# tarepan/QuickVC-official

Measured on AMD Instinct MI355X. Metric: audio samples/sec (16 kHz, 5 s utterances, batch 32 per GPU, whole hot path), higher is better.
Workload: dtype bf16x; 1 GPU; batch=32 offline VC, 5 s 16 kHz utterances, 1xMI355X per rank (BASELINE.json configs[2]); batch_per_gpu=32, frames=250, samples_per_utterance=80000, hipgraph=True, parallel_resblock_branches=False, parallelism=utterance-sharded x1, no per-step collective, batches_in_flight=2

## Files before the change

quickvc-official_amd/build.py:

```python
from __future__ import annotations

import os
import subprocess
import sys
from concurrent.futures import ThreadPoolExecutor

PKG = os.path.dirname(os.path.abspath(__file__))
ROOT = os.path.dirname(PKG)
CSRC = os.path.join(PKG, "csrc")
OBJ = os.path.join(PKG, "csrc", "_obj")
LIB = os.path.join(PKG, "libqvc_hip.so")
IO_LIB = os.path.join(PKG, "libqvc_io.so")
EMU_DIR = os.path.join(ROOT, "oracle", "_build")
EMU_LIB = os.path.join(EMU_DIR, "libqvc_emu.so")
HIPCC = os.environ.get("HIPCC", "/opt/rocm/bin/hipcc")
ARCH = "gfx950"

SOURCES = ["qvc_conv_f16.hip", "qvc_conv_bf16.hip", "qvc_wn2.hip", "qvc_chain.hip", "qvc_small.hip", "qvc_spk.hip", "qvc_mel.hip", "qvc_api.hip", "qvc_pack.cpp"]
HEADERS = ["qvc_plan.h", "qvc_kernels.h", "qvc_conv_impl.h", "qvc_wn2_impl.h", "qvc_chain_impl.h", "qvc_post_tail_impl.h", "qvc_tail_impl.h", "qvc_path.h", "qvc_stream.h", "qvc_pack_util.h", "qvc_launch_util.h"]


def _newer(target: str, deps) -> bool:
    if not os.path.exists(target):
        return False
    t = os.path.getmtime(target)
    return all(os.path.getmtime(d) <= t for d in deps)


def _run(cmd):
    res = subprocess.run(cmd, stdout=subprocess.PIPE, stderr=subprocess.STDOUT, text=True)
    if res.returncode != 0:
        raise RuntimeError("command failed: %s\n%s" % (" ".join(cmd), res.stdout))
    if "-c" in cmd and "-o" in cmd and cmd[cmd.index("-o") + 1].endswith(".o"):
        with open(cmd[cmd.index("-o") + 1][:-2] + ".remarks.txt", "w") as f:
            f.write(res.stdout)
    return res.stdout


def build_hip(force: bool = False, verbose: bool = False, variant: str = "") -> str:
    extra = {"": [], "sat": ["-DQVC_SATCOUNT"]}[variant]
    obj_dir = OBJ if not variant else os.path.join(OBJ, variant)
    lib = LIB if not variant else os.path.join(PKG, f"libqvc_hip_{variant}.so")
    os.makedirs(obj_dir, exist_ok=True)
    hdrs = [os.path.join(CSRC, h) for h in HEADERS] + [os.path.join(ROOT, "include", "qvc.h")]
    objs, jobs = [], []
    for src in SOURCES:
        s = os.path.join(CSRC, src)
        o = os.path.join(obj_dir, os.path.splitext(src)[0] + ".o")
        objs.append(o)
        if force or not _newer(o, [s] + hdrs):
            jobs.append([HIPCC, f"--offload-arch={ARCH}", "-O3", "-std=c++17", "-fPIC", "-Rpass-analysis=kernel-resource-usage"] + extra +
                        ["-c", s, "-o", o])
    if jobs:
        with ThreadPoolExecutor(max_workers=min(len(jobs), 6)) as ex:
            for out in ex.map(_run, jobs):
                if verbose and out.strip():
                    print(out)
    if jobs or not os.path.exists(lib):
        _run([HIPCC, f"--offload-arch={ARCH}", "-shared", "-fPIC", "-o", lib] + objs)
    return lib


def build_io(force: bool = False) -> str:
    src = os.path.join(CSRC, "qvc_io.cpp")
    hdr = os.path.join(ROOT, "include", "qvc_io.h")
    if force or not _newer(IO_LIB, [src, hdr]):
        _run(["g++", "-O2", "-std=c++17", "-fPIC", "-shared", "-pthread", "-o", IO_LIB, src])
    return IO_LIB


def build_emu(force: bool = False) -> str:
    os.makedirs(EMU_DIR, exist_ok=True)
    srcs = [os.path.join(ROOT, "oracle", "qvc_emu.cpp"), os.path.join(CSRC, "qvc_pack.cpp")]
    hdrs = [os.path.join(CSRC, h) for h in HEADERS] + [os.path.join(ROOT, "include", "qvc.h")]
    if force or not _newer(EMU_LIB, srcs + hdrs):
        _run(["g++", "-O2", "-std=c++17", "-fPIC", "-shared", "-o", EMU_LIB] + srcs)
    return EMU_LIB


if __name__ == "__main__":
    force = "--force" in sys.argv
    print(build_hip(force, verbose=True))
    print(build_hip(force, variant="sat"))
    print(build_io(force))
    print(build_emu(force))
```

quickvc-official_amd/csrc/qvc_conv_impl.h:

```cpp
#pragma once
#include <hip/hip_runtime.h>
#include <algorithm>
#include <type_traits>
#include <cstdlib>
#include "qvc_kernels.h"
#include "qvc_launch_util.h"

#ifndef QVC_SWZ_ROT
#define QVC_SWZ_ROT 1
#endif
namespace qvc {

typedef float f32x4 __attribute__((ext_vector_type(4)));
typedef _Float16 f16x8 __attribute__((ext_vector_type(8)));
typedef __bf16 bf16x8 __attribute__((ext_vector_type(8)));
typedef _Float16 f16x4 __attribute__((ext_vector_type(4)));
typedef __bf16 bf16x4 __attribute__((ext_vector_type(4)));

#ifdef QVC_SATCOUNT
static __device__ unsigned long long g_sat_count = 0;
#define QVC_SAT_READER(name)                                                                        \
  unsigned long long name(bool reset) {                                                             \
    unsigned long long v = 0, z = 0;                                                                \
    if (hipMemcpyFromSymbol(&v, HIP_SYMBOL(g_sat_count), 8) != hipSuccess) return ~0ull;            \
    if (reset && hipMemcpyToSymbol(HIP_SYMBOL(g_sat_count), &z, 8) != hipSuccess) return ~0ull;     \
    return v;                                                                                       \
  }
#endif

template <typename T> struct Op;
template <> struct Op<_Float16> {
  using frag = f16x8; using quad = f16x4;
  static __device__ __forceinline__ f32x4 mfma(frag a, frag b, f32x4 c) {
    return __builtin_amdgcn_mfma_f32_16x16x32_f16(a, b, c, 0, 0, 0);
  }
  static __device__ __forceinline__ _Float16 cvt(float f) {
#ifdef QVC_SATCOUNT
    if (__builtin_fabsf(f) > 65504.f) atomicAdd(&g_sat_count, 1ull);
#endif
    return (_Float16)__builtin_amdgcn_fmed3f(f, -65504.f, 65504.f);
  }
};
template <> struct Op<__bf16> {
  using frag = bf16x8; using quad = bf16x4;
  static __device__ __forceinline__ f32x4 mfma(frag a, frag b, f32x4 c) {
    return __builtin_amdgcn_mfma_f32_16x16x32_bf16(a, b, c, 0, 0, 0);
  }
  static __device__ __forceinline__ __bf16 cvt(float f) { return (__bf16)f; }
};

__device__ __forceinline__ float lrelu(float x, float slope) { return x > 0.f ? x : x * slope; }
__device__ __forceinline__ float fast_sigmoid(float x) {
  return __builtin_amdgcn_rcpf(1.f + __builtin_amdgcn_exp2f(-1.4426950408889634f * x));
}
__device__ __forceinline__ float fast_tanh(float x) {
  return 1.f - 2.f * __builtin_amdgcn_rcpf(__builtin_amdgcn_exp2f(2.8853900817779268f * x) + 1.f);
}

struct Swz { int sh, mask, rot; };
__device__ __forceinline__ Swz swz_mode(int cpr) {
  return (cpr & 15) == 0 ? Swz{0, QVC_SWZ_ROT ? 7 : 15, QVC_SWZ_ROT} : ((cpr & 7) == 0 ? Swz{0, 7, 0} : Swz{1, 3, 0});
}
__device__ __forceinline__ int swz(int row, Swz m) { return (row >> m.sh) & m.mask; }
__device__ __forceinline__ int rotc(int chunk, Swz m) {
  return m.rot ? ((chunk & ~15) | ((chunk & 1) << 3) | ((chunk >> 1) & 7)) : chunk;
}
template <typename B>
__device__ __forceinline__ B tile_at(B base, int row, int chunk, int rowbytes, Swz m) {
  return base + row * rowbytes + ((rotc(chunk, m) ^ swz(row, m)) << 4);
}

#define QVC_ZERO_ACC(acc) \
  _Pragma("unroll") for (auto& row_ : acc) { _Pragma("unroll") for (auto& e_ : row_) e_ = f32x4{0.f, 0.f, 0.f, 0.f}; }

__device__ __forceinline__ bool in_row(int ti, int Tlo, int Tin, int reflect, int& src) {
  if (reflect) { src = ti == Tlo ? Tlo + 1 : ti - 1; return ti >= Tlo && ti <= Tin; }
  src = ti;
  return ti >= Tlo && ti < Tin;
}

template <typename T>
__device__ __forceinline__ typename Op<T>::frag lrelu8(typename Op<T>::frag v, float slope) {
  typename Op<T>::frag r;
#pragma unroll
  for (int i = 0; i < 8; ++i) {
    const float f = (float)v[i];
    r[i] = (T)(f > 0.f ? f : f * slope);
  }
  return r;
}

template <>
__device__ __forceinline__ f16x8 lrelu8<_Float16>(f16x8 v, float slope) {
  f16x8 s;
#pragma unroll
  for (int i = 0; i < 8; ++i) s[i] = (_Float16)((float)v[i] * slope);
  return __builtin_elementwise_max(v, s);
}

template <typename T, typename TS>
__device__ __forceinline__ typename Op<T>::frag act8(typename Op<TS>::frag h, float slope) {
  if constexpr (std::is_same<T, TS>::value) {
    return lrelu8<T>(h, slope);
  } else {
    typename Op<T>::frag o;
#pragma unroll
    for (int e = 0; e < 8; ++e) o[e] = Op<T>::cvt(lrelu((float)h[e], slope));
    return o;
  }
}

template <typename T>
__device__ __forceinline__ typename Op<T>::frag cvt8(float4 v0, float4 v1) {
  using O = Op<T>;
  typename O::frag h;
  h[0] = O::cvt(v0.x); h[1] = O::cvt(v0.y); h[2] = O::cvt(v0.z); h[3] = O::cvt(v0.w);
  h[4] = O::cvt(v1.x); h[5] = O::cvt(v1.y); h[6] = O::cvt(v1.z); h[7] = O::cvt(v1.w);
  return h;
}
template <typename T>
__device__ __forceinline__ typename Op<T>::frag cvt8_lrelu(float4 v0, float4 v1, float slope) {
  return cvt8<T>(make_float4(lrelu(v0.x, slope), lrelu(v0.y, slope), lrelu(v0.z, slope), lrelu(v0.w, slope)),
                 make_float4(lrelu(v1.x, slope), lrelu(v1.y, slope), lrelu(v1.z, slope), lrelu(v1.w, slope)));
}

template <typename T>
__device__ __forceinline__ typename Op<T>::quad pack4_lrelu(f32x4 a, float4 b, float slope) {
  using O = Op<T>;
  typename O::quad h;
  h[0] = O::cvt(lrelu(a[0] + b.x, slope)); h[1] = O::cvt(lrelu(a[1] + b.y, slope));
  h[2] = O::cvt(lrelu(a[2] + b.z, slope)); h[3] = O::cvt(lrelu(a[3] + b.w, slope));
  return h;
}
template <typename T>
__device__ __forceinline__ typename Op<T>::quad pack4_res(f32x4 a, float4 b, typename Op<T>::quad r) {
  using O = Op<T>;
  typename O::quad h;
  h[0] = O::cvt(a[0] + b.x + (float)r[0]); h[1] = O::cvt(a[1] + b.y + (float)r[1]);
  h[2] = O::cvt(a[2] + b.z + (float)r[2]); h[3] = O::cvt(a[3] + b.w + (float)r[3]);
  return h;
}
template <typename T>
__device__ __forceinline__ typename Op<T>::frag pack8_lrelu(f32x4 a0, float4 b0, f32x4 a1, float4 b1, float slope) {
  const typename Op<T>::quad lo = pack4_lrelu<T>(a0, b0, slope), hi = pack4_lrelu<T>(a1, b1, slope);
  return __builtin_shufflevector(lo, hi, 0, 1, 2, 3, 4, 5, 6, 7);
}
template <typename T>
__device__ __forceinline__ typename Op<T>::frag pack8_res(f32x4 a0, float4 b0, f32x4 a1, float4 b1, typename Op<T>::frag r) {
  using quad = typename Op<T>::quad;
  const quad lo = pack4_res<T>(a0, b0, __builtin_shufflevector(r, r, 0, 1, 2, 3));
  const quad hi = pack4_res<T>(a1, b1, __builtin_shufflevector(r, r, 4, 5, 6, 7));
  return __builtin_shufflevector(lo, hi, 0, 1, 2, 3, 4, 5, 6, 7);
}

template <typename T>
__device__ __forceinline__ typename Op<T>::quad gate4(f32x4 t, f32x4 s, float4 bt, float4 bs) {
  using O = Op<T>;
  typename O::quad o;
  o[0] = O::cvt(fast_tanh(t[0] + bt.x) * fast_sigmoid(s[0] + bs.x));
  o[1] = O::cvt(fast_tanh(t[1] + bt.y) * fast_sigmoid(s[1] + bs.y));
  o[2] = O::cvt(fast_tanh(t[2] + bt.z) * fast_sigmoid(s[2] + bs.z));
  o[3] = O::cvt(fast_tanh(t[3] + bt.w) * fast_sigmoid(s[3] + bs.w));
  return o;
}

#ifndef QVC_PF_CONV
#define QVC_PF_CONV 3
#endif
#ifdef QVC_ABLATE
#define QVC_ABL(bit) ((QVC_ABLATE >> (bit)) & 1)
#else
#define QVC_ABL(bit) 0
#endif
#ifdef QVC_STAMP
#define QVC_ST(slot) do { if (st_ && lane == 0) st_[slot] = __builtin_amdgcn_s_memtime(); } while (0)
#else
#define QVC_ST(slot) ((void)0)
#endif
#ifndef QVC_PF_WN
#define QVC_PF_WN 3
#endif
#ifndef QVC_PF_STACK
#define QVC_PF_STACK 3
#endif

template <typename T, int MF, int kPF, int AS = MF>
__device__ __forceinline__ void gemm_prime(typename Op<T>::frag (&ar)[kPF + 1][MF], const typename Op<T>::frag* ap, int nIt) {
#pragma unroll
  for (int u = 0; u < kPF; ++u)
    if (u < nIt) {
#pragma unroll
      for (int m = 0; m < MF; ++m) ar[u][m] = ap[((size_t)u * AS + m) * 64];
    }
}

template <typename T, int MF, int NF, int kPF, int AS = MF>
__device__ __forceinline__ void gemm_loop_primed(f32x4 (&acc)[MF][NF], typename Op<T>::frag (&ar)[kPF + 1][MF],
                                                 const typename Op<T>::frag* ap, int nIt, int KS, int dil,
                                                 const char* tile, int rowbytes, Swz sm, int colrow, int lq) {
  using O = Op<T>;
  using frag = typename O::frag;
  constexpr int RING = kPF + 1;
  static_assert(RING % 2 == 0, "the B double buffer needs an even ring");
  frag bf[2][NF];
  const int nstride = 16 * rowbytes;
  int pf = kPF < nIt ? kPF : nIt;
  int tap = 0, ks = 0;
  auto read_b = [&](frag (&dst)[NF]) {
    const int row0 = tap * dil + colrow;
    const char* bp = tile + row0 * rowbytes + ((rotc(ks * 4 + lq, sm) ^ swz(row0, sm)) << 4);
#pragma unroll
    for (int n = 0; n < NF; ++n) dst[n] = *reinterpret_cast<const frag*>(bp + n * nstride);
    if (++ks == KS) { ks = 0; ++tap; }
  };
  if (nIt > 0) read_b(bf[0]);
  for (int it0 = 0; it0 < nIt; it0 += RING) {
#pragma unroll
    for (int u = 0; u < RING; ++u) {
      const int it = it0 + u;
      if (it < nIt) {
        if (it + kPF < nIt && !QVC_ABL(5)) {
#pragma unroll
          for (int m = 0; m < MF; ++m) ar[(u + kPF) % RING][m] = ap[((size_t)pf * AS + m) * 64];
          ++pf;
        }
        if (it + 1 < nIt && !QVC_ABL(6)) read_b(bf[(u + 1) & 1]);
        __builtin_amdgcn_sched_barrier(0);
#pragma unroll
        for (int n = 0; n < NF; ++n)
#pragma unroll
          for (int m = 0; m < MF; ++m) acc[m][n] = O::mfma(ar[u][m], bf[u & 1][n], acc[m][n]);
        __builtin_amdgcn_sched_barrier(0);
      }
    }
  }
}

template <typename T, int MF, int NF, int kPF, int AS = MF>
__device__ __forceinline__ void gemm_loop(f32x4 (&acc)[MF][NF], const typename Op<T>::frag* ap, int nIt, int KS, int dil,
                                          const char* tile, int rowbytes, Swz sm, int colrow, int lq) {
  typename Op<T>::frag ar[kPF + 1][MF];
  gemm_prime<T, MF, kPF, AS>(ar, ap, nIt);
  gemm_loop_primed<T, MF, NF, kPF, AS>(acc, ar, ap, nIt, KS, dil, tile, rowbytes, sm, colrow, lq);
}

template <typename T, typename TS, int NTHR, typename Put, typename Mid>
__device__ __forceinline__ void stage_stream_tile(const TS* xb, int C, int cpr, int total, int t_base, int Tlo, int Tb, float slope,
                                                  int tid, Put&& put, Mid&& loads_issued) {
  constexpr int kU = 16;
  const int rstep = NTHR / cpr, cstep = NTHR - rstep * cpr;
  for (int base = tid; base < total; base += NTHR * kU) {
    uint4 v[kU];
    const int r_0 = base / cpr, c_0 = base - r_0 * cpr;
    int r = r_0, c8 = c_0;
#pragma unroll
    for (int u = 0; u < kU; ++u) {
      const int idx = base + u * NTHR;
      const int ti = t_base + r;
      v[u] = make_uint4(0u, 0u, 0u, 0u);
      if (idx < total && ti >= Tlo && ti < Tb && c8 * 8 < C) v[u] = *reinterpret_cast<const uint4*>(xb + (size_t)ti * C + c8 * 8);
      c8 += cstep; r += rstep;
      if (c8 >= cpr) { c8 -= cpr; ++r; }
    }
    r = r_0; c8 = c_0;
    loads_issued(base == tid);
#pragma unroll
    for (int u = 0; u < kU; ++u) {
      const int idx = base + u * NTHR;
      if (idx < total) {
        typename Op<TS>::frag h; __builtin_memcpy(&h, &v[u], 16);
        put(r, c8, v[u], act8<T, TS>(h, slope));
      }
      c8 += cstep; r += rstep;
      if (c8 >= cpr) { c8 -= cpr; ++r; }
    }
  }
}

template <typename T, int MF, int NF, int WM, int EPI, bool CL = false>
__global__ __launch_bounds__(256) void conv_mfma_kernel(const ConvArgs a) {
  using O = Op<T>;
  using frag = typename O::frag;
  extern __shared__ __attribute__((aligned(16))) char smem[];
  constexpr int WN = kWaves / WM;
  constexpr int NT = WN * NF * 16;

  const int tid = threadIdx.x, lane = tid & 63;
  const int wave = __builtin_amdgcn_readfirstlane(tid >> 6);
  const int wm = wave % WM, wn = wave / WM;
  const int b = blockIdx.y;
  const int q0 = blockIdx.x * NT;
  const int R = NT + (a.taps - 1) * a.dil;
  const int rowbytes = a.CinP * 2;
  const int cpr = a.CinP >> 3;
  const Swz sm = swz_mode(cpr);
  const int t_base = q0 - a.left;
  const int Tin = ragged_len(a.rg, b, a.T_in);
  const int Tlo = ragged_lo(a.rg, b);
  if (a.rg.lens && t_base >= Tin + a.reflect) return;

  constexpr int kU = 4;
  if (a.x_kind == XK_F32_FM) {
    const float* xb = static_cast<const float*>(a.x) + (size_t)b * a.x_bs + a.x_c0;
    const float slope = a.slope_in;
    const int total = R * cpr;
    for (int base = tid; base < total; base += 256 * kU) {
      float4 v0[kU], v1[kU];
      int dst[kU];
#pragma unroll
      for (int u = 0; u < kU; ++u) {
        const int idx = base + u * 256;
        const int r = idx / cpr, c8 = idx - r * cpr;
        const int ti = t_base + r;
        int src;
        const bool ok = in_row(ti, Tlo, Tin, a.reflect, src) && idx < total && (c8 * 8 < a.Cin);
        v0[u] = make_float4(0.f, 0.f, 0.f, 0.f); v1[u] = v0[u];
        if (ok) {
          const float4* p = reinterpret_cast<const float4*>(xb + (size_t)src * a.x_ts + c8 * 8);
          v0[u] = p[0]; v1[u] = p[1];
        }
        dst[u] = idx < total ? tile_at(0, r, c8, rowbytes, sm) : -1;
      }
#pragma unroll
      for (int u = 0; u < kU; ++u) {
        if (dst[u] < 0) continue;
        *reinterpret_cast<frag*>(smem + dst[u]) = cvt8_lrelu<T>(v0[u], v1[u], slope);
      }
    }
  } else if (a.x_kind == XK_OP_FM && a.x2) {
    const size_t boff = (size_t)b * a.x_bs + a.x_c0;
    const T* xb = static_cast<const T*>(a.x) + boff;
    const T* xb2 = static_cast<const T*>(a.x2) + boff;
    const T* xb3 = static_cast<const T*>(a.x3) + boff;
    const float slope = a.slope_in;
    const int total = R * cpr;
    for (int base = tid; base < total; base += 256 * kU) {
      uint4 v1[kU], v2[kU], v3[kU];
      int dst[kU];
#pragma unroll
      for (int u = 0; u < kU; ++u) {
        const int idx = base + u * 256;
        const int r = idx / cpr, c8 = idx - r * cpr;
        const int ti = t_base + r;
        int src;
        const bool ok = in_row(ti, Tlo, Tin, a.reflect, src) && idx < total && (c8 * 8 < a.Cin);
        v1[u] = make_uint4(0u, 0u, 0u, 0u); v2[u] = v1[u]; v3[u] = v1[u];
        if (ok) {
          const size_t o = (size_t)src * a.x_ts + c8 * 8;
          v1[u] = *reinterpret_cast<const uint4*>(xb + o);
          v2[u] = *reinterpret_cast<const uint4*>(xb2 + o);
          v3[u] = *reinterpret_cast<const uint4*>(xb3 + o);
        }
        dst[u] = idx < total ? tile_at(0, r, c8, rowbytes, sm) : -1;
      }
#pragma unroll
      for (int u = 0; u < kU; ++u) {
        if (dst[u] < 0) continue;
        frag h1, h2, h3, h;
        __builtin_memcpy(&h1, &v1[u], 16); __builtin_memcpy(&h2, &v2[u], 16); __builtin_memcpy(&h3, &v3[u], 16);
#pragma unroll
        for (int i = 0; i < 8; ++i)
          h[i] = O::cvt(lrelu(((float)h1[i] + (float)h2[i] + (float)h3[i]) * (1.f / 3.f), slope));
        *reinterpret_cast<frag*>(smem + dst[u]) = h;
      }
    }
  } else if (a.x_kind == XK_OP_FM) {
    const T* xb = static_cast<const T*>(a.x) + (size_t)b * a.x_bs + a.x_c0;
    const int total = R * cpr;
    for (int base = tid; base < total; base += 256 * kU * 2) {
      uint4 v[kU * 2];
      int dst[kU * 2];
#pragma unroll
      for (int u = 0; u < kU * 2; ++u) {
        const int idx = base + u * 256;
        const int r = idx / cpr, c8 = idx - r * cpr;
        const int ti = t_base + r;
        int src;
        const bool ok = idx < total && in_row(ti, Tlo, Tin, 0, src) && (c8 * 8 < a.Cin);
        v[u] = make_uint4(0u, 0u, 0u, 0u);
        if (ok) v[u] = *reinterpret_cast<const uint4*>(xb + (size_t)src * a.x_ts + c8 * 8);
        dst[u] = idx < total ? tile_at(0, r, c8, rowbytes, sm) : -1;
      }
#pragma unroll
      for (int u = 0; u < kU * 2; ++u)
        if (dst[u] >= 0) {
          if (a.slope_in != 1.f) {
            frag h; __builtin_memcpy(&h, &v[u], 16);
            h = lrelu8<T>(h, a.slope_in);
            *reinterpret_cast<frag*>(smem + dst[u]) = h;
          } else {
            *reinterpret_cast<uint4*>(smem + dst[u]) = v[u];
          }
        }
    }
  } else {
    constexpr int kCM = 32;
    const float* xb = static_cast<const float*>(a.x) + (size_t)b * a.x_bs;
    const float slope = a.slope_in;
    const int total = R * a.CinP;
    for (int base = tid; base < total; base += 256 * kCM) {
      float v[kCM];
      int dst[kCM];
#pragma unroll
      for (int u = 0; u < kCM; ++u) {
        const int idx = base + u * 256;
        const int c = idx / R, r = idx - c * R;
        const int ti = t_base + r;
        v[u] = 0.f;
        if (idx < total && c < a.Cin && ti >= Tlo && ti < Tin) v[u] = xb[(size_t)c * a.x_ts + ti];
        dst[u] = idx < total ? tile_at(0, r, c >> 3, rowbytes, sm) + (c & 7) * 2 : -1;
      }
#pragma unroll
      for (int u = 0; u < kCM; ++u)
        if (dst[u] >= 0) *reinterpret_cast<T*>(smem + dst[u]) = O::cvt(lrelu(v[u], slope));
    }
  }
  __syncthreads();

  const int lrow = lane & 15, lq = lane >> 4;
  const int chunk_lo = CL ? 0 : (int)blockIdx.z, chunk_hi = CL ? a.nchunk : chunk_lo + 1;
  for (int chunk = chunk_lo; chunk < chunk_hi; ++chunk) {
  f32x4 acc[MF][NF];
  QVC_ZERO_ACC(acc);

  const frag* ap = static_cast<const frag*>(a.w) + ((size_t)(chunk * WM + wm) * a.nIt * MF) * 64 + lane;
  int it0 = 0;
  if (a.up_s > 1 && a.ksize > 0) {
    const int ph0 = ((chunk * WM + wm) * MF * 16) / a.Cout;
    const int real = ph0 < a.up_s ? (a.ksize - ph0 + a.up_s - 1) / a.up_s : 0;
    const int tap0 = a.taps - (real < a.taps ? real : a.taps);
    it0 = tap0 * a.KS;
  }
  gemm_loop<T, MF, NF, QVC_PF_CONV>(acc, ap + (size_t)it0 * MF * 64, a.nIt - it0, a.KS, a.dil, smem, rowbytes, sm,
                                    wn * (NF * 16) + lrow + (it0 / a.KS) * a.dil, lq);

  const int qw = q0 + wn * (NF * 16);
  if constexpr (EPI == EPI_GAU) {
    static_assert(EPI != EPI_GAU || MF % 2 == 0, "GAU epilogue pairs fragments");
    constexpr int HF = MF / 2;
    const int H = a.gau_H;
    const float* bb = a.bbias + (size_t)b * a.bbias_bs;
#pragma unroll
    for (int f = 0; f < HF; ++f) {
      const int ch0 = ((chunk * WM + wm) * HF + f) * 16 + lq * 4;
      if (ch0 >= H) continue;
      const float4 bt = *reinterpret_cast<const float4*>(bb + ch0);
      const float4 bs = *reinterpret_cast<const float4*>(bb + H + ch0);
      T* yb = static_cast<T*>(a.y16) + (size_t)b * a.y16_bs + ch0;
#pragma unroll
      for (int n = 0; n < NF; ++n) {
        const int q = qw + n * 16 + lrow;
        if (q < a.Nq) {
          *reinterpret_cast<typename O::quad*>(yb + (size_t)q * a.y16_ts) = gate4<T>(acc[f][n], acc[HF + f][n], bt, bs);
        }
      }
    }
  } else if constexpr (EPI == EPI_SAMPLE) {
    static_assert(EPI != EPI_SAMPLE || MF % 2 == 0, "paired rows");
    constexpr int HF = MF / 2;
    const int C = a.gau_H;
#pragma unroll
    for (int f = 0; f < HF; ++f) {
      const int ch0 = ((chunk * WM + wm) * HF + f) * 16 + lq * 4;
      if (ch0 >= C) continue;
      const float4 bm = *reinterpret_cast<const float4*>(a.bias + ch0);
      const float4 bl = *reinterpret_cast<const float4*>(a.bias + C + ch0);
      const float* nb = a.noise + (size_t)b * a.noise_bs + (size_t)ch0 * a.noise_ts;
      float* zb = a.y32 + (size_t)b * a.y32_bs + ch0;
#pragma unroll
      for (int n = 0; n < NF; ++n) {
        const int q = qw + n * 16 + lrow;
        if (q < a.Nq) {
          const f32x4 mu = acc[f][n], ls = acc[HF + f][n];
          const float n0 = nb[q], n1 = nb[(size_t)a.noise_ts + q], n2 = nb[2 * (size_t)a.noise_ts + q], n3 = nb[3 * (size_t)a.noise_ts + q];
          *reinterpret_cast<float4*>(zb + (size_t)q * a.y32_ts) =
              make_float4((mu[0] + bm.x) + n0 * expf(ls[0] + bl.x), (mu[1] + bm.y) + n1 * expf(ls[1] + bl.y),
                          (mu[2] + bm.z) + n2 * expf(ls[2] + bl.z), (mu[3] + bm.w) + n3 * expf(ls[3] + bl.w));
        }
      }
    }
  } else {
  bool packed = false;
  if constexpr (MF % 2 == 0) if (a.lp) {
    packed = true;
    const int v0 = (chunk * WM + wm) * MF * 16 + lq * 4 * MF;
    if (v0 < a.M) {
      int ph = 0, co = v0;
      if (a.up_s > 1) { ph = v0 / a.Cout; co = v0 - ph * a.Cout; }
      float4 bias[MF];
#pragma unroll
      for (int m = 0; m < MF; ++m) {
        bias[m] = make_float4(0.f, 0.f, 0.f, 0.f);
        if (a.bias) bias[m] = *reinterpret_cast<const float4*>(a.bias + v0 + m * 4);
        if (a.bbias) {
          const float4 bb = *reinterpret_cast<const float4*>(a.bbias + (size_t)b * a.bbias_bs + v0 + m * 4);
          bias[m].x += bb.x; bias[m].y += bb.y; bias[m].z += bb.z; bias[m].w += bb.w;
        }
      }
      T* yb = static_cast<T*>(a.y16) + (size_t)b * a.y16_bs + co;
#pragma unroll
      for (int n = 0; n < NF; ++n) {
        const int q = qw + n * 16 + lrow;
        const int o = q * a.up_s + ph - a.up_p;
        if (q >= a.Nq || o < 0 || o >= a.T_out) continue;
        frag h[MF / 2];
#pragma unroll
        for (int m = 0; m < MF; m += 2) h[m >> 1] = pack8_lrelu<T>(acc[m][n], bias[m], acc[m + 1][n], bias[m + 1], a.slope_out);
#pragma unroll
        for (int k2 = 0; k2 < MF / 2; ++k2) *reinterpret_cast<frag*>(yb + (size_t)o * a.y16_ts + k2 * 8) = h[k2];
      }
    }
  }
  if (!packed) {
#pragma unroll
    for (int m = 0; m < MF; ++m) {
      const int v = ((chunk * WM + wm) * MF + m) * 16 + lq * 4;
      if (v >= a.M) continue;
      int ph = 0, co = v;
      if (a.up_s > 1) { ph = v / a.Cout; co = v - ph * a.Cout; }
      float4 bias = make_float4(0.f, 0.f, 0.f, 0.f);
      if (a.bias) bias = *reinterpret_cast<const float4*>(a.bias + v);
      if (a.bbias) {
        const float4 bb = *reinterpret_cast<const float4*>(a.bbias + (size_t)b * a.bbias_bs + v);
        bias.x += bb.x; bias.y += bb.y; bias.z += bb.z; bias.w += bb.w;
      }
#pragma unroll
      for (int n = 0; n < NF; ++n) {
        const int q = qw + n * 16 + lrow;
        const int o = q * a.up_s + ph - a.up_p;
        if (q >= a.Nq || o < 0 || o >= a.T_out) continue;
        float4 val = make_float4(acc[m][n][0] + bias.x, acc[m][n][1] + bias.y, acc[m][n][2] + bias.z, acc[m][n][3] + bias.w);
        if (a.y32b && v >= a.split) {
          float* p = a.y32b + (size_t)b * a.y32_bs + (size_t)o * a.y32_ts + (v - a.split);
          float4 old = *reinterpret_cast<float4*>(p);
          old.x += val.x; old.y += val.y; old.z += val.z; old.w += val.w;
          *reinterpret_cast<float4*>(p) = old;
          continue;
        }
        if (a.res) {
          const float4 rr = *reinterpret_cast<const float4*>(a.res + (size_t)b * a.res_bs + (size_t)o * a.res_ts + a.res_c0 + co);
          val.x = rr.x + a.res_sign * val.x; val.y = rr.y + a.res_sign * val.y;
          val.z = rr.z + a.res_sign * val.z; val.w = rr.w + a.res_sign * val.w;
        }
        if (a.res16) {
          const typename O::quad rr = *reinterpret_cast<const typename O::quad*>(
              static_cast<const T*>(a.res16) + (size_t)b * a.res_bs + (size_t)o * a.res_ts + co);
          val.x = (float)rr[0] + a.res_sign * val.x; val.y = (float)rr[1] + a.res_sign * val.y;
          val.z = (float)rr[2] + a.res_sign * val.z; val.w = (float)rr[3] + a.res_sign * val.w;
        }
        if (a.y32) {
          float* p = a.y32 + (size_t)b * a.y32_bs + (size_t)o * a.y32_ts + a.y32_c0 + co;
          float4 out = make_float4(val.x * a.y_scale, val.y * a.y_scale, val.z * a.y_scale, val.w * a.y_scale);
          if (a.y_accum) {
            const float4 old = *reinterpret_cast<const float4*>(p);
            out.x += old.x; out.y += old.y; out.z += old.z; out.w += old.w;
          }
          if (v + 4 <= a.M) *reinterpret_cast<float4*>(p) = out;
          else { p[0] = out.x; if (v + 1 < a.M) p[1] = out.y; if (v + 2 < a.M) p[2] = out.z; }
        }
        if (a.y16) {
          typename O::quad h;
          h[0] = O::cvt(lrelu(val.x, a.slope_out)); h[1] = O::cvt(lrelu(val.y, a.slope_out));
          h[2] = O::cvt(lrelu(val.z, a.slope_out)); h[3] = O::cvt(lrelu(val.w, a.slope_out));
          *reinterpret_cast<typename O::quad*>(static_cast<T*>(a.y16) + (size_t)b * a.y16_bs + (size_t)o * a.y16_ts + co) = h;
        }
      }
    }
  }
  }
  }
}


template <typename T, int MF, int NF, int WM, int NWV, typename TS = T>
__global__ __launch_bounds__(NWV * 64) void rbpair_kernel(const PairArgs3 A) {
  using O = Op<T>;
  using frag = typename O::frag;
  using quad = typename O::quad;
  using OS = Op<TS>;
  using sfrag = typename OS::frag;
  using squad = typename OS::quad;
  extern __shared__ __attribute__((aligned(16))) char smem[];
  constexpr int WN = NWV / WM;
  constexpr int NTHR = NWV * 64;
  constexpr int NF1 = NF + 1;
  constexpr int NT = WN * NF * 16;
  constexpr int N1P = WN * NF1 * 16;
  constexpr bool kWide = MF % 2 == 0;

  const int tid = threadIdx.x, lane = tid & 63;
  const int wave = __builtin_amdgcn_readfirstlane(tid >> 6);
  const int wm = wave % WM, wn = wave / WM;
  const int lrow = lane & 15, lq = lane >> 4;
  const int b = blockIdx.y;
  const int nj = A.n;
  const int chain = nj > 1 ? (A.chain_major ? (int)blockIdx.z : (int)(blockIdx.x % (unsigned)nj)) : 0;
  const int tile = (nj > 1 && !A.chain_major) ? (int)(blockIdx.x / (unsigned)nj) : (int)blockIdx.x;
  const int q0 = tile * NT;
  PairArgs a = A.p[0];
  if (chain == 1) a = A.p[1];
  if (chain == 2) a = A.p[2];
  const int h2 = (a.k - 1) / 2, h1 = h2 * a.dil;
  const int Rx = N1P + 2 * h1;
  const int rowbytes = a.CP * 2;
  const int cpr = a.CP >> 3;
  const Swz sm = swz_mode(cpr);
  const TS* xb = static_cast<const TS*>(a.x) + (size_t)b * a.bs;
  const int cb = wm * MF * 16 + lq * 4 * MF;
  const int Tb = ragged_len(A.rg, b, a.T);
  const int Tlo = ragged_lo(A.rg, b);
  if (q0 >= Tb) return;
#ifdef QVC_STAMP
  unsigned long long* st_ = (A.stamps && wave == 0) ? A.stamps + (((size_t)blockIdx.z * gridDim.y + blockIdx.y) * gridDim.x + blockIdx.x) * 64 : nullptr;
#endif
  QVC_ST(0);
#ifdef QVC_STAMP
  if (st_ && lane == 0) st_[11] = __builtin_amdgcn_s_memrealtime();
#endif

  if (!QVC_ABL(0)) {
    stage_stream_tile<T, TS, NTHR>(xb, a.C, cpr, Rx * cpr, q0 - h2 - h1, Tlo, Tb, a.slope, tid,
        [&](int r, int c8, const uint4&, frag o) { *reinterpret_cast<frag*>(tile_at(smem, r, c8, rowbytes, sm)) = o; },
        [&](bool first) {
#ifdef QVC_STAMP
          if (first) {
            QVC_ST(8);
            asm volatile("s_waitcnt vmcnt(15)" ::: "memory");
            QVC_ST(9);
          }
#endif
        });
  }
  QVC_ST(10);
  __syncthreads();
  QVC_ST(1);

  {
    f32x4 acc[MF][NF1];
    QVC_ZERO_ACC(acc);
    const frag* ap = static_cast<const frag*>(a.w1) + ((size_t)wm * a.nIt * MF) * 64 + lane;
    if (!QVC_ABL(1)) gemm_loop<T, MF, NF1, QVC_PF_CONV>(acc, ap, a.nIt, a.KS, a.dil, smem, rowbytes, sm, wn * (NF1 * 16) + lrow, lq);
    QVC_ST(2);
    float4 bias[MF];
#pragma unroll
    for (int m = 0; m < MF; ++m) bias[m] = *reinterpret_cast<const float4*>(a.b1 + cb + m * 4);
    __syncthreads();
    QVC_ST(3);
#pragma unroll
    for (int n = 0; n < NF1; ++n) {
      const int jr = wn * (NF1 * 16) + n * 16 + lrow;
      const int f = q0 - h2 + jr;
      const bool inside = f >= Tlo && f < Tb;
      if constexpr (kWide) {
#pragma unroll
        for (int m = 0; m < MF; m += 2) {
          const int v = cb + m * 4;
          if (v >= a.CP) continue;
          frag h;
          if (inside && v < a.C) {
            h = pack8_lrelu<T>(acc[m][n], bias[m], acc[m + 1][n], bias[m + 1], a.slope);
          } else {
#pragma unroll
            for (int e = 0; e < 8; ++e) h[e] = (T)0.f;
          }
          *reinterpret_cast<frag*>(tile_at(smem, jr, v >> 3, rowbytes, sm)) = h;
        }
      } else {
#pragma unroll
        for (int m = 0; m < MF; ++m) {
          const int v = cb + m * 4;
          if (v >= a.CP) continue;
          quad h;
          if (inside && v < a.C) {
            h = pack4_lrelu<T>(acc[m][n], bias[m], a.slope);
          } else {
            h[0] = h[1] = h[2] = h[3] = (T)0.f;
          }
          *reinterpret_cast<quad*>(tile_at(smem, jr, v >> 3, rowbytes, sm) + (v & 7) * 2) = h;
        }
      }
    }
  }
  __syncthreads();
  QVC_ST(4);

  {
    f32x4 acc[MF][NF];
    QVC_ZERO_ACC(acc);
    const frag* ap = static_cast<const frag*>(a.w2) + ((size_t)wm * a.nIt * MF) * 64 + lane;
    if (!QVC_ABL(2)) gemm_loop<T, MF, NF, QVC_PF_CONV>(acc, ap, a.nIt, a.KS, 1, smem, rowbytes, sm, wn * (NF * 16) + lrow, lq);
    QVC_ST(5);
    float4 bias[MF];
#pragma unroll
    for (int m = 0; m < MF; ++m) bias[m] = *reinterpret_cast<const float4*>(a.b2 + cb + m * 4);
    const TS* xres = static_cast<const TS*>(a.x) + (size_t)b * a.bs;
    TS* yb = static_cast<TS*>(a.y) + (size_t)b * a.bs;
    const int qw = q0 + wn * (NF * 16) + lrow;
    if constexpr (kWide) {
      uint4 rr[MF / 2][NF];
#pragma unroll
      for (int m = 0; m < MF; m += 2) {
        const int v = cb + m * 4;
#pragma unroll
        for (int n = 0; n < NF; ++n) {
          const int q = qw + n * 16;
          const bool ok = v < a.C && q < Tb && !QVC_ABL(3);
          rr[m / 2][n] = *reinterpret_cast<const uint4*>(xres + (size_t)(ok ? q : 0) * a.C + (ok ? v : 0));
        }
      }
#pragma unroll
      for (int m = 0; m < MF; m += 2) {
        const int v = cb + m * 4;
        if (v >= a.C || (QVC_ABL(3) && acc[0][0][0] != 12345.f)) continue;
#pragma unroll
        for (int n = 0; n < NF; ++n) {
          const int q = qw + n * 16;
          if (q >= Tb) continue;
          sfrag r8; __builtin_memcpy(&r8, &rr[m / 2][n], 16);
          *reinterpret_cast<sfrag*>(yb + (size_t)q * a.C + v) = pack8_res<TS>(acc[m][n], bias[m], acc[m + 1][n], bias[m + 1], r8);
        }
      }
    } else {
      squad rr[MF][NF];
#pragma unroll
      for (int m = 0; m < MF; ++m) {
        const int v = cb + m * 4;
#pragma unroll
        for (int n = 0; n < NF; ++n) {
          const int q = qw + n * 16;
          const bool ok = v < a.C && q < Tb && !QVC_ABL(3);
          rr[m][n] = *reinterpret_cast<const squad*>(xres + (size_t)(ok ? q : 0) * a.C + (ok ? v : 0));
        }
      }
#pragma unroll
      for (int m = 0; m < MF; ++m) {
        const int v = cb + m * 4;
        if (v >= a.C || (QVC_ABL(3) && acc[0][0][0] != 12345.f)) continue;
#pragma unroll
        for (int n = 0; n < NF; ++n) {
          const int q = qw + n * 16;
          if (q >= Tb) continue;
          *reinterpret_cast<squad*>(yb + (size_t)q * a.C + v) = pack4_res<TS>(acc[m][n], bias[m], rr[m][n]);
        }
      }
    }
#ifdef QVC_STAMP
    __builtin_amdgcn_s_waitcnt(0);
#endif
    QVC_ST(6);
#ifdef QVC_STAMP
    if (st_ && lane == 0) st_[12] = __builtin_amdgcn_s_memrealtime();
#endif
  }
}


template <typename T, int NF, bool LAST, int WV>
__global__ __launch_bounds__(WV * 64) void wn_layer_kernel(const WnArgs a) {
  using O = Op<T>;
  using frag = typename O::frag;
  using quad = typename O::quad;
  extern __shared__ __attribute__((aligned(16))) char smem[];
  constexpr int FW = 1;
  constexpr int NT = NF * 16;
  constexpr int MF1 = 2 * FW, MF2 = LAST ? FW : 2 * FW;

  const int tid = threadIdx.x, lane = tid & 63, NTH = blockDim.x;
  const int wm = __builtin_amdgcn_readfirstlane(tid >> 6);
  const int lrow = lane & 15, lq = lane >> 4;
  const int b = blockIdx.y;
  const int q0 = blockIdx.x * NT;
  const int halo = a.taps - 1, left = halo / 2;
  const int R = NT + halo;
  const int rowbytes = a.HP * 2;
  const int cpr = a.HP >> 3;
  const Swz sm = swz_mode(cpr);
  char* acts = smem + R * rowbytes;
  const float* xb = a.x_in + (size_t)b * a.bs;
  const int Tb = ragged_len(a.rg, b, a.T), Tlo = ragged_lo(a.rg, b);
  if (q0 >= Tb) return;

  if (!QVC_ABL(0)) {
    const int total = R * cpr;
    constexpr int kU = 4;
    for (int base = tid; base < total; base += NTH * kU) {
      float4 v0[kU], v1[kU];
      int dst[kU];
#pragma unroll
      for (int u = 0; u < kU; ++u) {
        const int idx = base + u * NTH;
        const int r = idx / cpr, c8 = idx - r * cpr;
        const int ti = q0 - left + r;
        const bool ok = idx < total && ti >= Tlo && ti < Tb && (c8 * 8 < a.H);
        v0[u] = make_float4(0.f, 0.f, 0.f, 0.f); v1[u] = v0[u];
        if (ok) {
          const float4* p = reinterpret_cast<const float4*>(xb + (size_t)ti * a.H + c8 * 8);
          v0[u] = p[0]; v1[u] = p[1];
        }
        dst[u] = idx < total ? tile_at(0, r, c8, rowbytes, sm) : -1;
      }
#pragma unroll
      for (int u = 0; u < kU; ++u) {
        if (dst[u] < 0) continue;
        *reinterpret_cast<frag*>(smem + dst[u]) = cvt8<T>(v0[u], v1[u]);
      }
    }
  }
  __syncthreads();

  {
    f32x4 acc[MF1][NF];
    QVC_ZERO_ACC(acc);
    const frag* ap = static_cast<const frag*>(a.w_in) + ((size_t)wm * a.nIt1 * MF1) * 64 + lane;
    if (!QVC_ABL(1)) gemm_loop<T, MF1, NF, QVC_PF_WN>(acc, ap, a.nIt1, a.KS, 1, smem, rowbytes, sm, lrow, lq);
    const float* bb = a.bbias + (size_t)b * a.bbias_bs;
#pragma unroll
    for (int f = 0; f < FW; ++f) {
      const int ch0 = (wm * FW + f) * 16 + lq * 4;
      if (ch0 >= a.HP) continue;
      float4 bt = make_float4(0.f, 0.f, 0.f, 0.f), bs = bt;
      if (ch0 < a.H) { bt = *reinterpret_cast<const float4*>(bb + ch0); bs = *reinterpret_cast<const float4*>(bb + a.H + ch0); }
#pragma unroll
      for (int n = 0; n < NF; ++n) {
        const int j = n * 16 + lrow;
        quad o;
        if (ch0 < a.H) {
          o = gate4<T>(acc[f][n], acc[FW + f][n], bt, bs);
        } else {
          o[0] = o[1] = o[2] = o[3] = (T)0.f;
        }
        *reinterpret_cast<quad*>(tile_at(acts, j, ch0 >> 3, rowbytes, sm) + (ch0 & 7) * 2) = o;
      }
    }
  }
  __syncthreads();

  {
    f32x4 acc[MF2][NF];
    QVC_ZERO_ACC(acc);
    const frag* ap = static_cast<const frag*>(a.w_rs) + ((size_t)wm * a.KS * MF2) * 64 + lane;
    if (!QVC_ABL(2)) gemm_loop<T, MF2, NF, QVC_PF_WN>(acc, ap, a.KS, a.KS, 1, acts, rowbytes, sm, lrow, lq);
    float4 xin[FW][NF], oin[FW][NF];
#pragma unroll
    for (int f = 0; f < FW; ++f) {
      const int ch0 = (wm * FW + f) * 16 + lq * 4;
#pragma unroll
      for (int n = 0; n < NF; ++n) {
        const int q = q0 + n * 16 + lrow;
        const bool ok = ch0 < a.H && q < Tb && !QVC_ABL(3);
        const size_t off = (size_t)b * a.bs + (size_t)q * a.H + ch0;
        xin[f][n] = make_float4(0.f, 0.f, 0.f, 0.f); oin[f][n] = xin[f][n];
        if (ok) {
          if constexpr (!LAST) xin[f][n] = *reinterpret_cast<const float4*>(a.x_in + off);
          oin[f][n] = *reinterpret_cast<const float4*>(a.oacc + off);
        }
      }
    }
#pragma unroll
    for (int f = 0; f < FW; ++f) {
      const int ch0 = (wm * FW + f) * 16 + lq * 4;
      if (ch0 >= a.H || QVC_ABL(3)) continue;
      const float4 b0 = *reinterpret_cast<const float4*>(a.b_rs + ch0);
      float4 b1 = make_float4(0.f, 0.f, 0.f, 0.f);
      if constexpr (!LAST) b1 = *reinterpret_cast<const float4*>(a.b_rs + a.H + ch0);
#pragma unroll
      for (int n = 0; n < NF; ++n) {
        const int q = q0 + n * 16 + lrow;
        if (q >= Tb) continue;
        const size_t off = (size_t)b * a.bs + (size_t)q * a.H + ch0;
        float4 sk;
        if constexpr (!LAST) {
          const float4 xi = xin[f][n];
          *reinterpret_cast<float4*>(a.x_out + off) = make_float4(xi.x + acc[f][n][0] + b0.x, xi.y + acc[f][n][1] + b0.y,
                                                                  xi.z + acc[f][n][2] + b0.z, xi.w + acc[f][n][3] + b0.w);
          sk = make_float4(acc[FW + f][n][0] + b1.x, acc[FW + f][n][1] + b1.y, acc[FW + f][n][2] + b1.z, acc[FW + f][n][3] + b1.w);
        } else {
          sk = make_float4(acc[f][n][0] + b0.x, acc[f][n][1] + b0.y, acc[f][n][2] + b0.z, acc[f][n][3] + b0.w);
        }
        float4 o = oin[f][n];
        o.x += sk.x; o.y += sk.y; o.z += sk.z; o.w += sk.w;
        *reinterpret_cast<float4*>(a.oacc + off) = o;
      }
    }
  }
}


template <typename T, int NF, int PM, int WV>
__global__ __launch_bounds__(WV * 64) void wn_stack_kernel(const WnStackArgs a) {
  using O = Op<T>;
  using frag = typename O::frag;
  using quad = typename O::quad;
  extern __shared__ __attribute__((aligned(16))) char smem[];
  constexpr int FW = 1;
  constexpr int NB = NF * 16;
  constexpr int MF = 2 * FW;
  constexpr int OUTF = NF == 2 ? 16 : kWnOutFrames;
  constexpr int OLO = NF > 3 ? 1 : 0, ON = NF == 2 ? 2 : 3;

  const int tid = threadIdx.x, lane = tid & 63, NTH = blockDim.x;
  const int wm = __builtin_amdgcn_readfirstlane(tid >> 6);
  const int lrow = lane & 15, lq = lane >> 4;
  const int b = blockIdx.y;
  const int q0 = blockIdx.x * OUTF;
#ifdef QVC_STAMP
  unsigned long long* const st_ = a.stamps ? a.stamps + ((size_t)(blockIdx.y * gridDim.x + blockIdx.x) * 16 + wm) * 32 : nullptr;
  if (st_ && lane == 0) st_[27] = __builtin_amdgcn_s_memrealtime();
#endif
  QVC_ST(0);
  const int Tb = ragged_len(a.rg, b, a.T);
  const int Tlo = ragged_lo(a.rg, b);
  if (q0 >= Tb) return;
  const int left = (a.taps - 1) / 2;
  const int halo = left * a.layers;
  const int w0 = q0 - halo;
  const int rowbytes = a.HP * 2;
  const int cpr = a.HP >> 3;
  const Swz sm = swz_mode(cpr);
  const int R = NB + a.taps - 1;
  char* acts = smem + R * rowbytes;

  for (int i = tid; i < (R * rowbytes) >> 4; i += NTH) reinterpret_cast<uint4*>(smem)[i] = make_uint4(0u, 0u, 0u, 0u);

  f32x4 xr[FW][NF], outr[FW][ON];
  if (a.w_pre) {
    const int pcpr = a.pre_KS * 4;
    for (int i = tid; i < (NB * rowbytes) >> 4; i += NTH) reinterpret_cast<uint4*>(acts)[i] = make_uint4(0u, 0u, 0u, 0u);
    __syncthreads();
    const float* zb = a.z + (size_t)b * a.z_bs + a.pre_c0;
    for (int idx = tid; idx < NB * pcpr; idx += NTH) {
      const int r = idx / pcpr, c8 = idx - r * pcpr;
      const int q = w0 + r;
      if (q >= Tlo && q < Tb && c8 * 8 < a.pre_cin) {
        const float4* p = reinterpret_cast<const float4*>(zb + (size_t)q * a.z_ts + c8 * 8);
        *reinterpret_cast<frag*>(tile_at(acts, r, c8, rowbytes, sm)) = cvt8<T>(p[0], p[1]);
      }
    }
    __syncthreads();
    f32x4 pacc[FW][NF];
    QVC_ZERO_ACC(pacc);
    const frag* app = static_cast<const frag*>(a.w_pre) + ((size_t)wm * a.pre_KS * FW) * 64 + lane;
    gemm_loop<T, FW, NF, QVC_PF_STACK>(pacc, app, a.pre_KS, a.pre_KS, 1, acts, rowbytes, sm, lrow, lq);
#pragma unroll
    for (int f = 0; f < FW; ++f) {
      const int ch0 = (wm * FW + f) * 16 + lq * 4;
      float4 bp = make_float4(0.f, 0.f, 0.f, 0.f);
      if (ch0 < a.H) bp = *reinterpret_cast<const float4*>(a.b_pre + ch0);
#pragma unroll
      for (int n = 0; n < NF; ++n) {
        const int q = w0 + n * 16 + lrow;
        const bool in = ch0 < a.H && q >= Tlo && q < Tb;
        xr[f][n] = in ? f32x4{pacc[f][n][0] + bp.x, pacc[f][n][1] + bp.y, pacc[f][n][2] + bp.z, pacc[f][n][3] + bp.w}
                      : f32x4{0.f, 0.f, 0.f, 0.f};
      }
    }
  }
#pragma unroll
  for (int f = 0; f < FW; ++f) {
    const int ch0 = (wm * FW + f) * 16 + lq * 4;
#pragma unroll
    for (int n = 0; n < NF; ++n) {
      const int q = w0 + n * 16 + lrow;
      float4 v = make_float4(0.f, 0.f, 0.f, 0.f);
      if (!a.w_pre) {
        if (ch0 < a.H && q >= Tlo && q < Tb) v = *reinterpret_cast<const float4*>(a.x0 + (size_t)b * a.bs + (size_t)q * a.H + ch0);
        xr[f][n] = f32x4{v.x, v.y, v.z, v.w};
      }
      if (n >= OLO && n < OLO + ON) {
        float4 o = make_float4(0.f, 0.f, 0.f, 0.f);
        if (a.accum && ch0 < a.H && q >= q0 && q < q0 + OUTF && q < Tb)
          o = *reinterpret_cast<const float4*>(a.out + (size_t)b * a.bs + (size_t)q * a.H + ch0);
        outr[f][n - OLO] = f32x4{o.x, o.y, o.z, o.w};
      }
    }
  }
  __syncthreads();
  auto put_x = [&]() {
#pragma unroll
    for (int f = 0; f < FW; ++f) {
      const int ch0 = (wm * FW + f) * 16 + lq * 4;
      if (ch0 >= a.H) continue;
#pragma unroll
      for (int n = 0; n < NF; ++n) {
        const int r = n * 16 + lrow + left;
        quad h;
        h[0] = O::cvt(xr[f][n][0]); h[1] = O::cvt(xr[f][n][1]); h[2] = O::cvt(xr[f][n][2]); h[3] = O::cvt(xr[f][n][3]);
        *reinterpret_cast<quad*>(tile_at(smem, r, ch0 >> 3, rowbytes, sm) + (ch0 & 7) * 2) = h;
      }
    }
  };
  put_x();
  __syncthreads();
  QVC_ST(1);
// ... 404 lines not shown
```

Measured before the change: 1.462 billion samples/s.

## Use branch-free ring-buffered GEMM loop in rbpair kernel and set occupancy bounds

Adds gemm_loop_free, a software-pipelined MFMA loop that keeps a ring of prefetched weight fragments and double-buffered LDS B fragments. Prefetch indices are clamped to the last iteration and the tap/ks advance is written without branches, so the main loop runs without per-iteration conditionals and a short epilogue handles the remainder. The rbpair kernel uses this loop for both convolutions and gets a min-waves-per-SIMD launch bound from an estimated register count, which may force register limits or spills. The build also keeps the assembly for the conv sources so it can be inspected.

```diff
diff --git a/quickvc-official_amd/build.py b/quickvc-official_amd/build.py
--- a/quickvc-official_amd/build.py
+++ b/quickvc-official_amd/build.py
@@ -1,5 +1,6 @@
 from __future__ import annotations
 
+import glob
 import os
 import subprocess
 import sys
@@ -17,6 +18,7 @@
 ARCH = "gfx950"
 
 SOURCES = ["qvc_conv_f16.hip", "qvc_conv_bf16.hip", "qvc_wn2.hip", "qvc_chain.hip", "qvc_small.hip", "qvc_spk.hip", "qvc_mel.hip", "qvc_api.hip", "qvc_pack.cpp"]
+ASM_SOURCES = ["qvc_conv_f16.hip", "qvc_conv_bf16.hip"]
 HEADERS = ["qvc_plan.h", "qvc_kernels.h", "qvc_conv_impl.h", "qvc_wn2_impl.h", "qvc_chain_impl.h", "qvc_post_tail_impl.h", "qvc_tail_impl.h", "qvc_path.h", "qvc_stream.h", "qvc_pack_util.h", "qvc_launch_util.h"]
 
 
@@ -34,6 +36,13 @@
     if "-c" in cmd and "-o" in cmd and cmd[cmd.index("-o") + 1].endswith(".o"):
         with open(cmd[cmd.index("-o") + 1][:-2] + ".remarks.txt", "w") as f:
             f.write(res.stdout)
+    if "-save-temps=obj" in cmd:
+        base = cmd[cmd.index("-o") + 1][:-2]
+        for tmp in glob.glob(glob.escape(base) + "-hip-*") + glob.glob(glob.escape(base) + "-host-*") + glob.glob(glob.escape(base) + ".hip-hip-*"):
+            if tmp.endswith(f"-{ARCH}.s"):
+                os.replace(tmp, base + ".s")
+            else:
+                os.remove(tmp)
     return res.stdout
 
 
@@ -48,9 +57,10 @@
         s = os.path.join(CSRC, src)
         o = os.path.join(obj_dir, os.path.splitext(src)[0] + ".o")
         objs.append(o)
-        if force or not _newer(o, [s] + hdrs):
+        keep_asm = src in ASM_SOURCES and not variant
+        if force or not _newer(o, [s] + hdrs) or (keep_asm and not os.path.exists(o[:-2] + ".s")):
             jobs.append([HIPCC, f"--offload-arch={ARCH}", "-O3", "-std=c++17", "-fPIC", "-Rpass-analysis=kernel-resource-usage"] + extra +
-                        ["-c", s, "-o", o])
+                        (["-save-temps=obj"] if keep_asm else []) + ["-c", s, "-o", o])
     if jobs:
         with ThreadPoolExecutor(max_workers=min(len(jobs), 6)) as ex:
             for out in ex.map(_run, jobs):
diff --git a/quickvc-official_amd/csrc/qvc_conv_impl.h b/quickvc-official_amd/csrc/qvc_conv_impl.h
--- a/quickvc-official_amd/csrc/qvc_conv_impl.h
+++ b/quickvc-official_amd/csrc/qvc_conv_impl.h
@@ -244,6 +244,66 @@
   gemm_loop_primed<T, MF, NF, kPF, AS>(acc, ar, ap, nIt, KS, dil, tile, rowbytes, sm, colrow, lq);
 }
 
+template <typename T, int MF, int NF, int kPF>
+__device__ __forceinline__ void gemm_loop_free(f32x4 (&acc)[MF][NF], const typename Op<T>::frag* ap, int nIt, int KS, int dil,
+                                               const char* tile, int rowbytes, Swz sm, int colrow, int lq) {
+  using O = Op<T>;
+  using frag = typename O::frag;
+  constexpr int RING = kPF + 1;
+  static_assert(RING % 2 == 0, "the B double buffer needs an even ring");
+  if (nIt <= 0) return;
+  const int last = nIt - 1;
+  frag ar[RING][MF];
+#pragma unroll
+  for (int u = 0; u < kPF; ++u) {
+    const int pu = u < last ? u : last;
+#pragma unroll
+    for (int m = 0; m < MF; ++m) ar[u][m] = ap[((size_t)pu * MF + m) * 64];
+  }
+  frag bf[2][NF];
+  const int nstride = 16 * rowbytes;
+  int tap = 0, ks = 0, bs = 0;
+  auto read_b = [&](frag (&dst)[NF]) {
+    const int row0 = tap * dil + colrow;
+    const char* bp = tile + row0 * rowbytes + ((rotc(ks * 4 + lq, sm) ^ swz(row0, sm)) << 4);
+#pragma unroll
+    for (int n = 0; n < NF; ++n) dst[n] = *reinterpret_cast<const frag*>(bp + n * nstride);
+    const int adv = bs < last ? 1 : 0;
+    bs += adv;
+    ks += adv;
+    const int wrap = ks == KS ? 1 : 0;
+    ks = wrap ? 0 : ks;
+    tap += wrap;
+  };
+  auto mfmas = [&](int u) {
+    __builtin_amdgcn_sched_barrier(0);
+#pragma unroll
+    for (int n = 0; n < NF; ++n)
+#pragma unroll
+      for (int m = 0; m < MF; ++m) acc[m][n] = O::mfma(ar[u][m], bf[u & 1][n], acc[m][n]);
+    __builtin_amdgcn_sched_barrier(0);
+  };
+  read_b(bf[0]);
+  const int nfree = nIt - nIt % RING;
+  for (int it0 = 0; it0 < nfree; it0 += RING) {
+#pragma unroll
+    for (int u = 0; u < RING; ++u) {
+      const int pf = it0 + u + kPF < last ? it0 + u + kPF : last;
+      if (!QVC_ABL(5))
+#pragma unroll
+        for (int m = 0; m < MF; ++m) ar[(u + kPF) % RING][m] = ap[((size_t)pf * MF + m) * 64];
+      if (!QVC_ABL(6)) read_b(bf[(u + 1) & 1]);
+      mfmas(u);
+    }
+  }
+#pragma unroll
+  for (int u = 0; u < RING - 1; ++u)
+    if (nfree + u < nIt) {
+      if (nfree + u + 1 < nIt) read_b(bf[(u + 1) & 1]);
+      mfmas(u);
+    }
+}
+
 template <typename T, typename TS, int NTHR, typename Put, typename Mid>
 __device__ __forceinline__ void stage_stream_tile(const TS* xb, int C, int cpr, int total, int t_base, int Tlo, int Tb, float slope,
                                                   int tid, Put&& put, Mid&& loads_issued) {
@@ -572,8 +632,12 @@
 }
 
 
+constexpr int pair_waves_per_simd(int MF, int NF) {
+  const int regs = 4 * (MF * (NF + 1) + 2 * (NF + 1) + (QVC_PF_CONV + 1) * MF) + 16;
+  return regs <= 168 ? 3 : regs <= 256 ? 2 : 1;
+}
 template <typename T, int MF, int NF, int WM, int NWV, typename TS = T>
-__global__ __launch_bounds__(NWV * 64) void rbpair_kernel(const PairArgs3 A) {
+__global__ __launch_bounds__(NWV * 64, pair_waves_per_simd(MF, NF)) void rbpair_kernel(const PairArgs3 A) {
   using O = Op<T>;
   using frag = typename O::frag;
   using quad = typename O::quad;
@@ -639,7 +703,7 @@
     f32x4 acc[MF][NF1];
     QVC_ZERO_ACC(acc);
     const frag* ap = static_cast<const frag*>(a.w1) + ((size_t)wm * a.nIt * MF) * 64 + lane;
-    if (!QVC_ABL(1)) gemm_loop<T, MF, NF1, QVC_PF_CONV>(acc, ap, a.nIt, a.KS, a.dil, smem, rowbytes, sm, wn * (NF1 * 16) + lrow, lq);
+    if (!QVC_ABL(1)) gemm_loop_free<T, MF, NF1, QVC_PF_CONV>(acc, ap, a.nIt, a.KS, a.dil, smem, rowbytes, sm, wn * (NF1 * 16) + lrow, lq);
     QVC_ST(2);
     float4 bias[MF];
 #pragma unroll
@@ -688,7 +752,7 @@
     f32x4 acc[MF][NF];
     QVC_ZERO_ACC(acc);
     const frag* ap = static_cast<const frag*>(a.w2) + ((size_t)wm * a.nIt * MF) * 64 + lane;
-    if (!QVC_ABL(2)) gemm_loop<T, MF, NF, QVC_PF_CONV>(acc, ap, a.nIt, a.KS, 1, smem, rowbytes, sm, wn * (NF * 16) + lrow, lq);
+    if (!QVC_ABL(2)) gemm_loop_free<T, MF, NF, QVC_PF_CONV>(acc, ap, a.nIt, a.KS, 1, smem, rowbytes, sm, wn * (NF * 16) + lrow, lq);
     QVC_ST(5);
     float4 bias[MF];
 #pragma unroll
```

New measurement: 1.483 billion samples/s, median of 6. 1.4% higher.
